# angeladai/sgnn

Measured on AMD Instinct MI355X. Metric: TSDF blocks/sec fwd+bwd (64^3@5% occ, bs32), higher is better.
Workload: dtype f32

## Files before the change

### include/sgnn_hip.h

```cpp
#ifndef SGNN_HIP_H
#define SGNN_HIP_H

#include <stdint.h>

#ifdef __cplusplus
extern "C" {
#endif

#define SGNN_OK 0
#define SGNN_EINVAL (-1)
#define SGNN_EHIP (-2)
#define SGNN_EOVERFLOW (-3)
#define SGNN_ENOWS (-4)

#define SGNN_STATUS_COORD_RANGE 1
#define SGNN_STATUS_DUPLICATE 2
#define SGNN_STATUS_OVERFLOW 4

typedef void *sgnn_stream_t;

const char *sgnn_last_error(void);
int sgnn_version(void);
const char *sgnn_arch(void);

// ... 40 lines not shown

#define SGNN_RULEBOOK_MULTI_MAX 4
int sgnn_rulebook_subm3_multi(int count, const uint64_t *const *keys, const int32_t *const *vals, const int64_t *caps,
                              const int32_t *const *coords, const int64_t *ns, int32_t *const *nbrs, const int64_t *lds,
                              const int64_t *const *n_devs, sgnn_stream_t stream);

int sgnn_rulebook_subm3_dense(const uint64_t *keys, const int32_t *vals, int64_t cap, const int32_t *coords, int64_t n,
                              int dim_z, int dim_y, int dim_x, int32_t *volume, int64_t volume_entries, int32_t *nbr,
                              int64_t ld, const int64_t *n_dev, sgnn_stream_t stream);
int sgnn_rulebook_subm3_volume(const int32_t *coords, int64_t n, int dim_z, int dim_y, int dim_x, int32_t *volume,
                               int64_t volume_entries, int32_t *nbr, int64_t ld, const int64_t *n_dev, int32_t *status,
                               sgnn_stream_t stream);

int64_t sgnn_down2_ws_bytes(int64_t nf);
int sgnn_rulebook_down2(const int32_t *fine_coords, int64_t nf, uint64_t *ckeys, int32_t *cvals,
                        int64_t ccap, int32_t *parent, int32_t *coarse_coords, int64_t *n_coarse,
                        void *ws, int64_t ws_bytes, sgnn_stream_t stream);
int sgnn_down2_tables(const int32_t *fine_coords, const int32_t *parent, int64_t nf,
                      int32_t *children, int64_t ldc, int64_t nc, int32_t *ptable, int64_t ldf,
                      const int64_t *nf_dev, const int64_t *nc_dev, sgnn_stream_t stream);

int64_t sgnn_down2_chain_ws_bytes(int64_t cap);
int sgnn_down2_chain(const int32_t *fine_coords, int64_t n0, const int64_t *n0_dev, int64_t cap, int depth,
                     void *const *ckeys, void *const *cvals, int64_t ccap, void *const *parent,
                     void *const *coarse_coords, int64_t *counts_dev, const int64_t *level_caps, int32_t *status,
                     void *ws, int64_t ws_bytes, sgnn_stream_t stream);

int64_t sgnn_down2_chain_tables_ws_bytes(int64_t cap, int depth);
int sgnn_down2_chain_tables(const int32_t *fine_coords, const int64_t *n0_dev, int64_t cap, int depth,
                            void *const *ckeys, void *const *cvals, int64_t ccap, void *const *parent,
                            void *const *coarse_coords, int64_t *counts_dev, const int64_t *level_caps,
                            void *const *children, void *const *ptable, int32_t *status, void *ws, int64_t ws_bytes,
                            sgnn_stream_t stream);

#define SGNN_CONV_TRANSPOSE_W 1
#define SGNN_CONV_FLIP_K 2
int sgnn_conv_fwd(const float *x, int64_t n_in, int cin, const float *w, int K, const int32_t *table,
                  int64_t ld, int64_t n_out, int cout, float *y, int flags, int in_shift,
                  sgnn_stream_t stream);

int sgnn_conv_fwd_ex(const float *x, int64_t n_in, int cin, const float *w, int K, const int32_t *table,
                     int64_t ld, int64_t n_out, int cout, float *y, int flags, int in_shift,
                     const int32_t *kmap, const int32_t *kadd, int in_mul, int groups, int table_rows,
                     sgnn_stream_t stream);
int sgnn_conv_bwd_weight_ex(const float *x, int64_t n_in, int cin, const float *dy, int cout,
                            const int32_t *table, int64_t ld, int K, int64_t n_out, float *dw, int in_shift,
                            const int32_t *kmap, const int32_t *kadd, int in_mul, int groups, int table_rows,
                            void *ws, int64_t ws_bytes, sgnn_stream_t stream);

int64_t sgnn_conv_stats_blocks(int64_t n_out);
int sgnn_conv_fwd_epi(const float *x, int64_t n_in, int cin, int64_t ldx, const float *w, int K,
                      const int32_t *table, int64_t ld, int64_t n_out, int cout, float *y, int64_t ldy, int flags,
                      const float *addend, int64_t ld_add, int stats, double *partial, const float *bn_x,
                      int64_t ld_bnx, const float *mean, const float *invstd, const float *gamma, const float *beta,
                      float leak, sgnn_stream_t stream);

int64_t sgnn_conv_bwd_weight_ws_bytes(int64_t n_out, int K, int cin, int cout);
int sgnn_conv_bwd_weight(const float *x, int64_t n_in, int cin, const float *dy, int cout,
                         const int32_t *table, int64_t ld, int K, int64_t n_out, float *dw, int in_shift, void *ws,
                         int64_t ws_bytes, sgnn_stream_t stream);

int sgnn_expand_weights(const float *w, int cin, int cout, float *wc, sgnn_stream_t stream);
int sgnn_expand_weights_bwd(const float *dwc, int cin, int cout, float *dw, sgnn_stream_t stream);

int64_t sgnn_bn_ws_bytes(int64_t n, int c);
int sgnn_bn_fwd(const float *x, int64_t n, int c, const float *gamma, const float *beta,
// ... 334 lines not shown
```

### sgnn_amd/_lib.py

```python
import ctypes
import os

import torch

_HERE = os.path.dirname(os.path.abspath(__file__))
LIB_PATH = os.environ.get('SGNN_LIB') or os.path.join(_HERE, 'lib', 'libsgnn_hip.so')

c_i32, c_i64, c_f32, c_vp, c_cp = ctypes.c_int, ctypes.c_int64, ctypes.c_float, ctypes.c_void_p, ctypes.c_char_p

PROTOTYPES = {
    'sgnn_last_error': (c_cp, []),
    'sgnn_version': (c_i32, []),
    'sgnn_arch': (c_cp, []),
    'sgnn_tune_set': (c_i64, [c_cp, c_i64]),
    'sgnn_tune_get': (c_i64, [c_cp]),
    'sgnn_tune_names': (c_cp, []),
    'sgnn_tune_current': (c_vp, []),
    'sgnn_hash_capacity': (c_i64, [c_i64]),
    'sgnn_coords_from_i64': (c_i32, [c_vp, c_i64, c_vp, c_vp, c_vp, c_vp]),
    'sgnn_coords_to_i64': (c_i32, [c_vp, c_i64, c_vp, c_vp, c_vp]),
    'sgnn_hash_build': (c_i32, [c_vp, c_i64, c_vp, c_vp, c_i64, c_vp, c_vp, c_vp]),
    'sgnn_hash_lookup': (c_i32, [c_vp, c_vp, c_i64, c_vp, c_i64, c_vp, c_vp, c_vp]),
    'sgnn_rulebook_subm3': (c_i32, [c_vp, c_vp, c_i64, c_vp, c_i64, c_vp, c_i64, c_vp, c_vp]),
    'sgnn_rulebook_subm3_multi': (c_i32, [c_i32, c_vp, c_vp, c_vp, c_vp, c_vp, c_vp, c_vp, c_vp, c_vp]),
    'sgnn_rulebook_subm3_dense': (c_i32, [c_vp, c_vp, c_i64, c_vp, c_i64, c_i32, c_i32, c_i32, c_vp, c_i64, c_vp, c_i64, c_vp, c_vp]),
    'sgnn_rulebook_subm3_volume': (c_i32, [c_vp, c_i64, c_i32, c_i32, c_i32, c_vp, c_i64, c_vp, c_i64, c_vp, c_vp, c_vp]),
    'sgnn_down2_ws_bytes': (c_i64, [c_i64]),
    'sgnn_rulebook_down2': (c_i32, [c_vp, c_i64, c_vp, c_vp, c_i64, c_vp, c_vp, c_vp, c_vp, c_i64, c_vp]),
    'sgnn_down2_chain_ws_bytes': (c_i64, [c_i64]),
    'sgnn_down2_chain': (c_i32, [c_vp, c_i64, c_vp, c_i64, c_i32, c_vp, c_vp, c_i64, c_vp, c_vp, c_vp, c_vp, c_vp, c_vp, c_i64, c_vp]),
    'sgnn_down2_chain_tables_ws_bytes': (c_i64, [c_i64, c_i32]),
    'sgnn_down2_chain_tables': (c_i32, [c_vp, c_vp, c_i64, c_i32, c_vp, c_vp, c_i64, c_vp, c_vp, c_vp, c_vp, c_vp, c_vp, c_vp, c_vp,
                                        c_i64, c_vp]),
    'sgnn_down2_tables': (c_i32, [c_vp, c_vp, c_i64, c_vp, c_i64, c_i64, c_vp, c_i64, c_vp, c_vp, c_vp]),
    'sgnn_conv_fwd': (c_i32, [c_vp, c_i64, c_i32, c_vp, c_i32, c_vp, c_i64, c_i64, c_i32, c_vp, c_i32, c_i32, c_vp]),
    'sgnn_conv_fwd_ex': (c_i32, [c_vp, c_i64, c_i32, c_vp, c_i32, c_vp, c_i64, c_i64, c_i32, c_vp, c_i32, c_i32, c_vp, c_vp, c_i32, c_i32, c_i32, c_vp]),
    'sgnn_conv_bwd_weight_ex': (c_i32, [c_vp, c_i64, c_i32, c_vp, c_i32, c_vp, c_i64, c_i32, c_i64, c_vp, c_i32, c_vp, c_vp, c_i32, c_i32, c_i32, c_vp, c_i64, c_vp]),
    'sgnn_conv_stats_blocks': (c_i64, [c_i64]),
    'sgnn_conv_fwd_epi': (c_i32, [c_vp, c_i64, c_i32, c_i64, c_vp, c_i32, c_vp, c_i64, c_i64, c_i32, c_vp, c_i64, c_i32, c_vp, c_i64, c_i32, c_vp, c_vp, c_i64, c_vp, c_vp, c_vp, c_vp, c_f32, c_vp]),
    'sgnn_conv_bwd_weight_ws_bytes': (c_i64, [c_i64, c_i32, c_i32, c_i32]),
    'sgnn_conv_bwd_weight': (c_i32, [c_vp, c_i64, c_i32, c_vp, c_i32, c_vp, c_i64, c_i32, c_i64, c_vp, c_i32, c_vp, c_i64, c_vp]),
    'sgnn_bn_ws_bytes': (c_i64, [c_i64, c_i32]),
    'sgnn_bn_fwd': (c_i32, [c_vp, c_i64, c_i32, c_vp, c_vp, c_vp, c_vp, c_f32, c_f32, c_i32, c_f32, c_vp, c_vp, c_vp, c_vp, c_i64, c_vp]),
    'sgnn_bn_bwd': (c_i32, [c_vp, c_vp, c_i64, c_i32, c_vp, c_vp, c_vp, c_vp, c_i32, c_f32, c_vp, c_vp, c_vp, c_vp, c_i64, c_vp]),
    'sgnn_bn_bwd_add': (c_i32, [c_vp, c_vp, c_i64, c_i32, c_vp, c_vp, c_vp, c_vp, c_i32, c_f32, c_vp, c_vp, c_vp, c_vp, c_vp, c_i64, c_vp]),
    'sgnn_bn_fwd_ex': (c_i32, [c_vp, c_i64, c_i64, c_i32, c_vp, c_vp, c_vp, c_vp, c_f32, c_f32, c_i32, c_f32, c_vp, c_vp, c_vp, c_i64, c_vp, c_i64, c_vp, c_i64, c_vp]),
    'sgnn_bn_bwd_ex': (c_i32, [c_vp, c_i64, c_vp, c_i64, c_i64, c_i32, c_vp, c_vp, c_vp, c_vp, c_i32, c_f32, c_vp, c_i64, c_vp, c_i64, c_vp, c_vp, c_vp, c_i64, c_vp, c_i64, c_vp]),
    'sgnn_copy_multi': (c_i32, [c_vp, c_vp, c_vp, c_i32, c_vp]),
    'sgnn_gather_rows': (c_i32, [c_vp, c_i32, c_vp, c_i64, c_vp, c_vp]),
    'sgnn_gather_rows_dn': (c_i32, [c_vp, c_i32, c_vp, c_vp, c_i64, c_vp, c_vp]),
    'sgnn_scatter_rows': (c_i32, [c_vp, c_i32, c_vp, c_i64, c_vp, c_i64, c_vp, c_vp]),
    'sgnn_gather_sum': (c_i32, [c_vp, c_i32, c_vp, c_i64, c_i32, c_i64, c_vp, c_vp]),
    'sgnn_repeat_rows': (c_i32, [c_vp, c_i32, c_i64, c_i32, c_vp, c_vp]),
    'sgnn_sum_groups': (c_i32, [c_vp, c_i32, c_i64, c_i32, c_vp, c_vp]),
    'sgnn_concat_rows': (c_i32, [c_vp, c_i32, c_vp, c_vp, c_i32, c_vp, c_i64, c_vp, c_vp]),
    'sgnn_concat_rows_bwd': (c_i32, [c_vp, c_i32, c_vp, c_i32, c_vp, c_i64, c_vp, c_i64, c_vp, c_i64, c_vp]),
    'sgnn_add': (c_i32, [c_vp, c_vp, c_i64, c_vp, c_vp]),
    'sgnn_expand8_coords': (c_i32, [c_vp, c_i64, c_vp, c_vp, c_vp]),
    'sgnn_expand8_coords_i64': (c_i32, [c_vp, c_i64, c_vp, c_vp, c_vp, c_vp]),
    'sgnn_dense_coords': (c_i32, [c_i32, c_i32, c_i32, c_i32, c_vp, c_vp]),
    'sgnn_compact_ws_bytes': (c_i64, [c_i64]),
    'sgnn_compact_sigmoid': (c_i32, [c_vp, c_i64, c_i64, c_vp, c_vp, c_vp, c_i64, c_vp]),
    'sgnn_compact_dense': (c_i32, [c_vp, c_i64, c_vp, c_i32, c_i32, c_i32, c_i32, c_vp, c_vp, c_vp, c_i64, c_vp]),
    'sgnn_compact_mask': (c_i32, [c_vp, c_i64, c_vp, c_vp, c_vp, c_i64, c_vp]),
    'sgnn_compact_sigmoid_cap': (c_i32, [c_vp, c_i64, c_i64, c_vp, c_vp, c_vp, c_i64, c_vp, c_vp, c_i64, c_vp]),
    'sgnn_compact_dense_cap': (c_i32, [c_vp, c_i64, c_vp, c_vp, c_i32, c_i32, c_i32, c_i32, c_vp, c_vp, c_i64, c_vp, c_vp, c_i64, c_vp]),
# ... 226 lines not shown
```

### sgnn_amd/csrc/grid_rules.hip

```cpp
#include <stdarg.h>
#include "common.h"

static thread_local char g_err[512] = "";

void sgnn_set_error(const char *fmt, ...) {
  va_list ap;
  va_start(ap, fmt);
  vsnprintf(g_err, sizeof(g_err), fmt, ap);
  va_end(ap);
}

SGNN_EXPORT const char *sgnn_last_error(void) { return g_err; }
SGNN_EXPORT int sgnn_version(void) { return 100; }
SGNN_EXPORT const char *sgnn_arch(void) { return "gfx950"; }

SGNN_EXPORT int64_t sgnn_hash_capacity(int64_t n) {
  const int64_t want = 4 * n < 262144 ? 4 * n : (2 * n > 262144 ? 2 * n : 262144);
  int64_t cap = 1024;
  while (cap < want) cap <<= 1;
  return cap;
}

__global__ __launch_bounds__(256) void k_coords_from_i64(const int64_t *__restrict__ locs, int64_t n,
                                                        int4 *__restrict__ coords, int32_t *status,
// ... 690 lines not shown
}

#define CHAIN_MAX_DEPTH 8

struct ChainScratch {
  int32_t *slot_of, *rank_at, *owner;
};

static int64_t chain_ws_bytes(int64_t cap, int64_t ccap, int slices) {
  const int64_t nblk = (cap + SCAN_BLOCK - 1) / SCAN_BLOCK;
  return (slices * (2 * cap + ccap) + nblk + 1) * (int64_t)sizeof(int32_t) + 256;
}

static int32_t *chain_ws_carve(void *ws, int64_t cap, int64_t ccap, int slices, ChainScratch *w) {
  int32_t *p = (int32_t *)ws;
  for (int l = 0; l < slices; ++l, p += 2 * cap + ccap) w[l] = ChainScratch{p, p + cap, p + 2 * cap};
  return p;
}

struct ChainInit {
  unsigned long long *ckeys[CHAIN_MAX_DEPTH];
  int32_t *owner[CHAIN_MAX_DEPTH];
  int32_t *rank_at[CHAIN_MAX_DEPTH];
  int64_t ccap, cap;
};

__device__ __forceinline__ void chain_init_rows(unsigned long long *__restrict__ ckeys, int32_t *__restrict__ owner,
                                                int64_t ccap, int32_t *__restrict__ rank_at, int64_t cap) {
  const int64_t stride = (int64_t)gridDim.x * 256;
  const int64_t top = ccap > cap ? ccap : cap;
  for (int64_t i = (int64_t)blockIdx.x * 256 + threadIdx.x; i < top; i += stride) {
    if (i < ccap) {
      ckeys[i] = ~0ull;
      owner[i] = 0x7FFFFFFF;
    }
    if (i < cap) rank_at[i] = -1;
  }
}

__global__ __launch_bounds__(256) void k_chain_init(unsigned long long *__restrict__ ckeys, int32_t *__restrict__ owner,
                                                   int64_t ccap, int32_t *__restrict__ rank_at, int64_t cap) {
  chain_init_rows(ckeys, owner, ccap, rank_at, cap);
}

__global__ __launch_bounds__(256) void k_chain_init_all(ChainInit a) {
  chain_init_rows(a.ckeys[blockIdx.y], a.owner[blockIdx.y], a.ccap, a.rank_at[blockIdx.y], a.cap);
}

__device__ __forceinline__ void chain_insert_rows(const int4 *__restrict__ fine, const int64_t *n_dev, int64_t n_host,
                                                  unsigned long long *__restrict__ ckeys,
                                                  int32_t *__restrict__ owner, uint64_t mask,
                                                  int32_t *__restrict__ slot_of) {
  const int64_t nf = sgnn_dyn_n(n_host, n_dev);
  int64_t i = (int64_t)blockIdx.x * 256 + threadIdx.x;
  const int64_t stride = (int64_t)gridDim.x * 256;
  for (; i < nf; i += stride) {
    const int4 c = fine[i];
    const uint64_t key = sgnn_pack_key(c.x >> 1, c.y >> 1, c.z >> 1, c.w);
    uint64_t slot = sgnn_hash64(key) & mask;
    while (true) {
      const unsigned long long prev = atomicCAS(&ckeys[slot], SGNN_EMPTY_KEY, (unsigned long long)key);
      if (prev == SGNN_EMPTY_KEY || prev == key) break;
      slot = (slot + 1) & mask;
    }
    atomicMin(&owner[slot], (int32_t)i);
    slot_of[i] = (int32_t)slot;
  }
}

// ... 124 lines not shown
  for (; i < iend; i += stride) {
    if (Tables && i >= nf) {
      down2_table_row<false>(i, true, fine, -1, nc, nullptr, children, ldc, ptable, ldf);
      continue;
    }
    const int32_t sl = slot_of[i];
    const int32_t p = rank_at[owner[sl]];
    if (rank_at[i] >= 0) cvals[sl] = p;
    if (Tables) down2_table_row<true>(i, false, fine, p, nc, parent, children, ldc, ptable, ldf);
    else parent[i] = p;
  }
}

__global__ __launch_bounds__(256) void k_chain_parent(const int64_t *n_dev, int64_t n_host,
                                                     const int32_t *__restrict__ owner,
                                                     const int32_t *__restrict__ rank_at,
                                                     const int32_t *__restrict__ slot_of,
                                                     int32_t *__restrict__ parent, int32_t *__restrict__ cvals) {
  chain_parent_rows<false>(nullptr, n_dev, n_host, owner, rank_at, slot_of, parent, cvals, nullptr, 0, nullptr, 0, nullptr, 0);
}

__global__ __launch_bounds__(256) void k_chain_parent_tables(ChainTables t) {
  chain_parent_rows<true>(t.fine, t.n_dev, t.n_host, t.owner, t.rank_at, t.slot_of, t.parent, t.cvals, t.nc_dev, t.nc_cap,
                          t.children, t.ldc, t.ptable, t.ldf);
}

__global__ __launch_bounds__(256) void k_chain_tables_insert(ChainTables t, unsigned long long *__restrict__ ckeys_next,
                                                            int32_t *__restrict__ owner_next, uint64_t mask,
                                                            int32_t *__restrict__ slot_of_next, const int4 *coarse,
                                                            int64_t n_host_next) {
  chain_parent_rows<true>(t.fine, t.n_dev, t.n_host, t.owner, t.rank_at, t.slot_of, t.parent, t.cvals, t.nc_dev, t.nc_cap,
                          t.children, t.ldc, t.ptable, t.ldf);
  chain_insert_rows(coarse, t.nc_dev, n_host_next, ckeys_next, owner_next, mask, slot_of_next);
}

static void chain_launch_init(const ChainInit &ini, int levels, hipStream_t s) {
  SGNN_LAUNCH(k_chain_init_all, dim3(sgnn_grid_for(ini.ccap, 256, 4096), levels), dim3(256), 0, s, ini);
}

static void chain_launch_insert(const int4 *fine, const int64_t *n_dev, int64_t n_host, int64_t cap, void *ckeys,
                                const ChainScratch &w, int64_t ccap, hipStream_t s) {
  SGNN_LAUNCH(k_chain_insert, dim3(sgnn_grid_for(cap, 256, 8192)), dim3(256), 0, s, fine, n_dev, n_host,
              (unsigned long long *)ckeys, w.owner, (uint64_t)(ccap - 1), w.slot_of);
}

static ScanInline chain_launch_count(const ChainScratch &w, const int64_t *n_dev, int64_t n_host, int64_t cap,
                                     int32_t *block_sums, int64_t *count, const ScanLimit &lim, hipStream_t s) {
  const int64_t nblk = (cap + SCAN_BLOCK - 1) / SCAN_BLOCK;
  SGNN_LAUNCH((k_scan_count<FlagOwner>), dim3((unsigned)nblk), dim3(256), 0, s, FlagOwner{w.slot_of, w.owner}, n_host,
              block_sums, n_dev);
  if (scan_inline_ok(nblk)) return ScanInline{nblk, count, lim};
  SGNN_LAUNCH(k_scan_block_sums, dim3(1), dim3(1024), 0, s, block_sums, nblk, count, lim);
  return kNoInline;
}

SGNN_EXPORT int64_t sgnn_down2_ws_bytes(int64_t nf) { return chain_ws_bytes(nf, sgnn_hash_capacity(nf), 1); }
SGNN_EXPORT int64_t sgnn_down2_chain_ws_bytes(int64_t cap) { return chain_ws_bytes(cap, sgnn_hash_capacity(cap), 1); }
SGNN_EXPORT int64_t sgnn_down2_chain_tables_ws_bytes(int64_t cap, int depth) {
  return chain_ws_bytes(cap, sgnn_hash_capacity(cap), depth);
}

static int chain_hip_result(const char *who, hipError_t e) {
  if (e == hipSuccess) return SGNN_OK;
  sgnn_set_error("%s: HIP error: %s", who, hipGetErrorString(e));
  return SGNN_EHIP;
}
// ... 34 lines not shown
                (const int32_t *)w.rank_at, (const int32_t *)w.slot_of, (int32_t *)parent[l], (int32_t *)cvals[l]);
    fine = (const int4 *)coarse_coords[l];
    n_dev = counts_dev + l;
    n_host = cap;
  }
  return chain_hip_result(who, hipGetLastError());
}

SGNN_EXPORT int sgnn_rulebook_down2(const int32_t *fine_coords, int64_t nf, uint64_t *ckeys, int32_t *cvals,
                                    int64_t ccap, int32_t *parent, int32_t *coarse_coords,
                                    int64_t *n_coarse, void *ws, int64_t ws_bytes, sgnn_stream_t stream) {
  SGNN_CHECK_ARG(nf >= 0 && n_coarse && ckeys && cvals);
  SGNN_CHECK_ARG(ccap >= 2 * nf && ccap >= 2 && (ccap & (ccap - 1)) == 0 && ccap < (1ll << 31));
  SGNN_CHECK_ARG(nf == 0 || (fine_coords && parent && coarse_coords));
  void *const k = ckeys, *const v = cvals, *const p = parent, *const c = coarse_coords;
  return down2_chain("sgnn_rulebook_down2", fine_coords, nf, nullptr, nf, 1, &k, &v, ccap, &p, &c, n_coarse, nullptr,
                     nullptr, ws, ws_bytes, (hipStream_t)stream);
}

SGNN_EXPORT int sgnn_down2_chain(const int32_t *fine_coords, int64_t n0, const int64_t *n0_dev, int64_t cap, int depth,
                                 void *const *ckeys, void *const *cvals, int64_t ccap, void *const *parent,
                                 void *const *coarse_coords, int64_t *counts_dev, const int64_t *level_caps,
                                 int32_t *status, void *ws, int64_t ws_bytes, sgnn_stream_t stream) {
  SGNN_CHECK_ARG(!level_caps || status);
  SGNN_CHECK_ARG(depth >= 1 && depth <= CHAIN_MAX_DEPTH && cap >= 0 && n0 >= 0 && n0 <= cap && counts_dev && ckeys &&
                 cvals && parent && coarse_coords);
  SGNN_CHECK_ARG(ccap >= 2 * cap && ccap >= 2 && (ccap & (ccap - 1)) == 0 && ccap < (1ll << 31));
  for (int l = 0; l < depth; ++l) SGNN_CHECK_ARG(ckeys[l] && (cap == 0 || (cvals[l] && parent[l] && coarse_coords[l])));
  SGNN_CHECK_ARG(cap == 0 || fine_coords);
  return down2_chain("sgnn_down2_chain", fine_coords, n0, n0_dev, cap, depth, ckeys, cvals, ccap, parent, coarse_coords,
                     counts_dev, level_caps, status, ws, ws_bytes, (hipStream_t)stream);
}

SGNN_EXPORT int sgnn_down2_chain_tables(const int32_t *fine_coords, const int64_t *n0_dev, int64_t cap, int depth,
                                        void *const *ckeys, void *const *cvals, int64_t ccap, void *const *parent,
                                        void *const *coarse_coords, int64_t *counts_dev, const int64_t *level_caps,
                                        void *const *children, void *const *ptable, int32_t *status, void *ws,
                                        int64_t ws_bytes, sgnn_stream_t stream) {
  hipStream_t s = (hipStream_t)stream;
  SGNN_CHECK_ARG(depth >= 1 && depth <= CHAIN_MAX_DEPTH && cap >= 1 && n0_dev && counts_dev && level_caps && status &&
                 ckeys && cvals && parent && coarse_coords && children && ptable && fine_coords);
  SGNN_CHECK_ARG(ccap >= 2 * cap && ccap >= 2 && (ccap & (ccap - 1)) == 0 && ccap < (1ll << 31));
  if (!ws || ws_bytes < chain_ws_bytes(cap, ccap, depth)) {
    sgnn_set_error("sgnn_down2_chain_tables: workspace too small");
    return SGNN_ENOWS;
  }
  ChainScratch w[CHAIN_MAX_DEPTH];
  int32_t *block_sums = chain_ws_carve(ws, cap, ccap, depth, w);
  ChainInit ini{};
  for (int l = 0; l < depth; ++l) {
    SGNN_CHECK_ARG(ckeys[l] && cvals[l] && parent[l] && coarse_coords[l] && children[l] && ptable[l] && level_caps[l] >= 1);
    ini.ckeys[l] = (unsigned long long *)ckeys[l];
    ini.owner[l] = w[l].owner;
    ini.rank_at[l] = w[l].rank_at;
  }
  ini.ccap = ccap;
  ini.cap = cap;
  chain_launch_init(ini, depth, s);
  const int4 *fine = (const int4 *)fine_coords;
  const int64_t *n_dev = n0_dev;
  int64_t fine_cap = cap;
  const int g = sgnn_grid_for(cap, 256, 8192);
  const bool merged = g_tune.chain_merged != 0;
  for (int l = 0; l < depth; ++l) {
    const int64_t ccap_l = level_caps[l] < cap ? level_caps[l] : cap;
    const int64_t ldc = ((ccap_l + 255) / 256) * 256, ldf = ((fine_cap + 255) / 256) * 256;
    if (l == 0 || !merged)
      chain_launch_insert(fine, n_dev, cap, cap, ckeys[l], w[l], ccap, s);
    const ScanInline si = chain_launch_count(w[l], n_dev, cap, cap, block_sums, counts_dev + l,
                                             ScanLimit{ccap_l, nullptr, 0, status}, s);
    SGNN_LAUNCH(k_chain_emit2, dim3((unsigned)((cap + SCAN_BLOCK - 1) / SCAN_BLOCK)), dim3(256), 0, s, fine,
                (const int32_t *)w[l].slot_of, (const int32_t *)w[l].owner, n_dev, cap, (const int32_t *)block_sums,
                (int4 *)coarse_coords[l], w[l].rank_at, (const int64_t *)(counts_dev + l), (int32_t *)children[l], ldc, si);
    const ChainTables t{fine, n_dev, cap, w[l].owner, w[l].rank_at, w[l].slot_of, (int32_t *)parent[l], (int32_t *)cvals[l],
                        counts_dev + l, ccap_l, (int32_t *)children[l], ldc, (int32_t *)ptable[l], ldf};
    if (merged && l + 1 < depth)
      SGNN_LAUNCH(k_chain_tables_insert, dim3(g), dim3(256), 0, s, t, (unsigned long long *)ckeys[l + 1], w[l + 1].owner,
                  (uint64_t)(ccap - 1), w[l + 1].slot_of, (const int4 *)coarse_coords[l], cap);
    else
      SGNN_LAUNCH(k_chain_parent_tables, dim3(g), dim3(256), 0, s, t);
    fine = (const int4 *)coarse_coords[l];
    n_dev = counts_dev + l;
    fine_cap = ccap_l;
  }
  SGNN_CHECK_LAUNCH();
  return SGNN_OK;
}

__global__ __launch_bounds__(256) void k_down2_tables(const int4 *__restrict__ fine,
                                                     const int32_t *__restrict__ parent, int64_t nf,
                                                     int32_t *__restrict__ children, int64_t ldc,
                                                     int32_t *__restrict__ ptable, int64_t ldf, int64_t nc,
                                                     const int64_t *nf_dev, const int64_t *nc_dev) {
  nf = sgnn_dyn_n(nf, nf_dev);
  nc = sgnn_dyn_n(nc, nc_dev);
  int64_t i = (int64_t)blockIdx.x * 256 + threadIdx.x;
  const int64_t stride = (int64_t)gridDim.x * 256;
  const int64_t iend = pad_end(nf, ldf);
  for (; i < iend; i += stride) {
    if (i >= nf)
      down2_table_row<false>(i, true, fine, -1, nc, nullptr, children, ldc, ptable, ldf);
    else
      down2_table_row<false>(i, false, fine, parent[i], nc, nullptr, children, ldc, ptable, ldf);
  }
}

SGNN_EXPORT int sgnn_down2_tables(const int32_t *fine_coords, const int32_t *parent, int64_t nf,
                                  int32_t *children, int64_t ldc, int64_t nc, int32_t *ptable, int64_t ldf,
                                  const int64_t *nf_dev, const int64_t *nc_dev, sgnn_stream_t stream) {
  hipStream_t s = (hipStream_t)stream;
  SGNN_CHECK_ARG(nf >= 0 && nc >= 0 && ldc >= nc && ldf >= nf);
  if (nc > 0) {
    SGNN_CHECK_ARG(children);
    if (nc_dev)
      SGNN_LAUNCH(k_fill_rows_dyn, dim3(sgnn_grid_for(8 * nc, 256, 4096)), dim3(256), 0, s, children, 8, ldc, nc, nc_dev);
    else
      if (sgnn_fill32(children, 0xFFFFFFFFu, 8 * ldc, s) != SGNN_OK) return SGNN_EHIP;
  }
  if (nf == 0) return SGNN_OK;
// ... 83 lines not shown
```

### sgnn_amd/model.py

```python
import os

import numpy as np
import torch
import torch.nn as nn
import torch.nn.functional as F

from . import scn
from .scn import functions as F_
from .scn import program as P_
from .scn.metadata import coords_from_locs
from .scn.sites import info, attach


STAGES = True
TEACHER_GEOMETRY_FIRST = os.environ.get('SGNN_TEACHER_GEOMETRY_FIRST', '1') != '0'


def _k4s2_maps():
    P, S = [], []
    for g in range(8):
        j = (g >> 2, (g >> 1) & 1, g & 1)
        for i_ in range(8):
            i = (i_ >> 2, (i_ >> 1) & 1, i_ & 1)
            k = [3 - 2 * i[a] - j[a] for a in range(3)]
# ... 587 lines not shown
        R = len(self.refinement)
        plan = F_.compact_sigmoid_plan(geo.coords, 2, int(geo.coords.shape[0]), geo.coords, 2 if runs[0] else 0, teacher[0])
        plans = [plan]
        for h in range(R):
            if not runs[h] or plan[1] == 0:
                plans.append(None)
                continue
            locs = plan[2]
            children = F_.expand8_coords(locs)
            attach(locs, children=children)
            plan = F_.compact_sigmoid_plan(children, 2, 8 * plan[1], children,
                                           self.refinement[h].plan_depth, teacher[h + 1])
            plans.append(plan)
        return plans

    def _forward_stages(self, feat_rows, occ_rows, skips, geo, loss_weights, runs, teacher=None, plans=None,
                        capacity=None):
        if not (self.pass_occ or self.pass_feats):
            return None
        R = len(self.refinement)
        if getattr(geo, 'coords_i64', None) is None:
            geo.coords_i64 = F_.coords_to_i64(geo.coords)
        outputs = [[geo.coords_i64, occ_rows]]
        n_all = occ_rows.shape[0]
        tv = (lambda h: None) if teacher is None else (lambda h: teacher[h])
        if plans is not None:
            sel, cnt, locs = plans[0]
        elif capacity is not None:
            sel, cnt, locs = F_.compact_capped(occ_rows.detach(), 2, n_all, geo.coords, 2 if runs[0] else 0, capacity, 0,
                                               tv(0))
        else:
            sel, cnt, locs = F_.compact_sigmoid_plan(occ_rows.detach(), 2, n_all, geo.coords, 2 if runs[0] else 0, tv(0))
        prev = (occ_rows if self.pass_occ else None, feat_rows if self.pass_feats else None, sel, locs, cnt)
        for h in range(R):
            if not runs[h]:
                outputs.append([[], []])
                continue
            if cnt == 0:
                outputs.append([[], []])
                continue
            ref = self.refinement[h]
            got = ref.stage(prev, skips[R - h] if self.use_skip_sparse else None)
            if got is None:
                return None if h == 0 else self._stage_fallback()
            y, out, coords_next = got
            outputs.append([F_.coords_to_i64(coords_next), out])
            if plans is not None:
                sel, cnt, locs = plans[h + 1]
            elif capacity is not None:
                sel, cnt, locs = F_.compact_capped(out.detach(), 2, out.shape[0], coords_next, ref.plan_depth, capacity,
                                                   h + 1, tv(h + 1))
            else:
                sel, cnt, locs = F_.compact_sigmoid_plan(out.detach(), 2, out.shape[0], coords_next, ref.plan_depth, tv(h + 1))
            prev = (y if ref.pass_feats else None, out if ref.pass_occ else None, sel, locs, cnt)
        if not runs[R]:
            return [[], []], outputs
        if cnt == 0:
            return [[], []], outputs
        sdf = self.surfacepred.stage(prev, skips[0] if self.use_skip_sparse else None)
        if sdf is None:
            return self._stage_fallback()
        return [F_.coords_to_i64(prev[3]), sdf], outputs

    @staticmethod
    def _stage_fallback():
        raise RuntimeError('sgnn_amd: a generative stage could not be compiled into a native program after an earlier '
                           'one was; set sgnn_amd.model.STAGES = False to run the per-module path')
```

### sgnn_amd/scn/functions.py

```python
import torch
from torch.autograd import Function

from .. import _lib
from .._lib import ptr
from .metadata import runtime
from .sites import info, attach

import os

CONV_TRANSPOSE_W = 1
CONV_FLIP_K = 2
FUSED_GLUE = os.environ.get('SGNN_FUSED_GLUE', '1') != '0'


_ws_cache = {}


def _ws_bytes(name, *args):
    k = (name,) + args
    v = _ws_cache.get(k)
    if v is None:
        if len(_ws_cache) > 4096:
            _ws_cache.clear()
        v = _ws_cache[k] = _lib.query(name, *args)
# ... 483 lines not shown
def compact_sigmoid_plan(logits, stride, n, coords_all, depth, teacher=None):
    from . import metadata as MD
    rt = runtime(logits.device)
    if not MD.CHAIN or depth < 1 or n == 0:
        if teacher is None:
            sel, cnt = compact_sigmoid(logits, stride, n)
        else:
            sel = torch.empty(max(n, 1), dtype=torch.int32, device=logits.device)
            wsb = _lib.query('sgnn_compact_ws_bytes', n)
            _compact_call(logits, stride, n, coords_all, sel, rt, rt.workspace(wsb), wsb, teacher)
            cnt = rt.read_count()
            sel = sel[:cnt]
        if MD.COUNT_LOG is not None:
            MD.COUNT_LOG.append(('gen', int(cnt), []))
        return sel, cnt, gather_coords(coords_all, sel, cnt)
    sel = torch.empty(n, dtype=torch.int32, device=logits.device)
    wsb = _lib.query('sgnn_compact_ws_bytes', n)
    ws = rt.workspace(wsb)
    _compact_call(logits, stride, n, coords_all, sel, rt, ws, wsb, teacher)
    locs_cap = torch.empty(n, 4, dtype=torch.int32, device=logits.device)
    _lib.call('sgnn_gather_rows_dn', ptr(coords_all), 4, ptr(sel), ptr(rt.state), n, ptr(locs_cap))
    _inherit_bounds(locs_cap, coords_all)
    chain = MD.PendingChain(locs_cap, 0, True, depth)
    host = rt.read_counts()
    count = int(host[0])
    locs = _inherit_bounds(locs_cap[:count], coords_all)
    if MD.COUNT_LOG is not None:
        MD.COUNT_LOG.append(('gen', count, [int(v) for v in host[2:2 + chain.depth]]))
    if count:
        attach(locs, plan=chain.finalize(count, host))
    return sel[:count], count, locs


def compact_capped(logits, stride, n_all, coords_all, depth, capacity, g, teacher=None):
    from . import metadata as MD
    dev = coords_all.device
    rt = runtime(dev)
    K, pyr_caps = capacity.gen[g]
    cnt2 = capacity.kept2(g)
    n_cnt = info(coords_all).cnt
    sel = torch.empty(max(n_all, 1), dtype=torch.int32, device=dev)
    wsb = _lib.query('sgnn_compact_ws_bytes', n_all)
    ws = rt.workspace(wsb)
    kept, kept8 = cnt2[0:1], cnt2[1:2]
    locs = _inherit_bounds(torch.empty(K, 4, dtype=torch.int32, device=dev), coords_all)
    if FUSED_GLUE:
        if teacher is None:
            _lib.call('sgnn_compact_sigmoid_cap_locs', ptr(logits), stride, n_all, ptr(n_cnt), ptr(coords_all), ptr(sel),
                      ptr(locs), ptr(cnt2), K, ptr(rt.status32), ptr(ws), wsb)
        else:
            B, _, d0, d1, d2 = (int(v) for v in teacher.shape)
            _lib.call('sgnn_compact_dense_cap_locs', ptr(coords_all), n_all, ptr(n_cnt), ptr(teacher), B, d0, d1, d2,
                      ptr(sel), ptr(locs), ptr(cnt2), K, ptr(rt.status32), ptr(ws), wsb)
    else:
        if teacher is None:
            _lib.call('sgnn_compact_sigmoid_cap', ptr(logits), stride, n_all, ptr(n_cnt), ptr(sel), ptr(cnt2), K,
                      ptr(rt.status32), ptr(ws), wsb)
        else:
            B, _, d0, d1, d2 = (int(v) for v in teacher.shape)
            _lib.call('sgnn_compact_dense_cap', ptr(coords_all), n_all, ptr(n_cnt), ptr(teacher), B, d0, d1, d2, ptr(sel),
                      ptr(cnt2), K, ptr(rt.status32), ptr(ws), wsb)
        _lib.call('sgnn_gather_rows_dn', ptr(coords_all), 4, ptr(sel), ptr(kept), K, ptr(locs))
    attach(locs, cnt=kept, cnt8=kept8)
    if depth >= 1:
        depth = min(depth, len(pyr_caps))
        chain = MD.PendingChain(locs, K, True, depth, n0_cnt=kept, counts=capacity.pyr_counts(g, depth),
                                level_caps=pyr_caps)
        attach(locs, plan=chain.finalize_capped())
    return sel, K, locs


def compact_mask(mask_u8, n):
    rt = runtime(mask_u8.device)
    sel = torch.empty(max(n, 1), dtype=torch.int32, device=mask_u8.device)
    wsb = _lib.query('sgnn_compact_ws_bytes', n)
    ws = rt.workspace(wsb)
    _lib.call('sgnn_compact_mask', ptr(mask_u8), n, ptr(sel), ptr(rt.state), ptr(ws), wsb)
    count = rt.read_count()
    return sel[:count], count


def _inherit_bounds(coords, parent, scale=1):
    b = info(parent).bounds
    if b is not None:
        attach(coords, bounds=(int(b[0]), int(b[1]) * scale, int(b[2]) * scale, int(b[3]) * scale))
    return coords


def gather_coords(coords32, sel, m):
    out = torch.empty(m, 4, dtype=torch.int32, device=coords32.device)
    _lib.call('sgnn_gather_rows', ptr(coords32), 4, ptr(sel), m, ptr(out))
    return _inherit_bounds(out, coords32)


def expand8_coords(coords32, with_i64=False):
    n = coords32.shape[0]
    out = torch.empty(8 * n, 4, dtype=torch.int32, device=coords32.device)
    parent = info(coords32)
    cnt, o64 = parent.cnt, None
    if with_i64 and FUSED_GLUE:
# ... 27 lines not shown
```

### sgnn_amd/scn/metadata.py

```python
import numpy as np
import os
import threading
from contextlib import nullcontext as _nullcontext

import torch

from .. import _lib
from .._lib import ptr
from .sites import info, attach, carry


SIDE_LANE = os.environ.get('SGNN_SIDE_LANE', '1') != '0'
SIDE_PRIORITY = int(os.environ.get('SGNN_SIDE_PRIORITY', '0'))
SIDE_PYRAMID = os.environ.get('SGNN_SIDE_PYRAMID', '1') != '0'
PYRAMID_LANE = 2


class _Runtime(object):

    def __init__(self, device):
        self.device = device
        self.ws = torch.empty(1 << 20, dtype=torch.uint8, device=device)
        self.state = torch.zeros(8, dtype=torch.int64, device=device)
        self.status32 = self.state[1:2].view(torch.int32)
        self.syncs = 0

    def index_volume(self):
        if getattr(self, '_volume', None) is None:
            self._volume = torch.full((INDEX_VOLUME_ENTRIES,), -1, dtype=torch.int32, device=self.device)
        return self._volume

    def workspace(self, nbytes):
        if self.ws.numel() < nbytes:
            self.ws = torch.empty(int(nbytes * 1.5) + 256, dtype=torch.uint8, device=self.device)
        return self.ws

    def pyramid_stream(self):
        if getattr(self, '_side_stream', None) is None:
            self._side_stream = torch.cuda.Stream(device=self.device, priority=SIDE_PRIORITY)
            self._side_ws = None
        self._pyr_stream = self._side_stream
        return self._pyr_stream

    def side_lane(self, nbytes):
        if not SIDE_LANE:
            if getattr(self, '_side_on', False):
                _lib.query('sgnn_prog_set_side_stream', None, None, 0)
                self._side_on = False
# ... 154 lines not shown
        return out if self.cnt is None else attach(out, cnt=self.cnt)


class Down2(object):
    ready = None

    def __init__(self, fine, coarse, parent, children, ldc, ptable, ldf):
        self.fine, self.coarse = fine, coarse
        self.parent, self.children, self.ldc, self.ptable, self.ldf = parent, children, ldc, ptable, ldf


def build_down2(fine):
    rt = runtime(fine.device)
    nf, dev = fine.n, fine.device
    ccap = _lib.query('sgnn_hash_capacity', nf)
    ckeys = torch.empty(ccap, dtype=torch.int64, device=dev)
    cvals = torch.empty(ccap, dtype=torch.int32, device=dev)
    parent = torch.empty(max(nf, 1), dtype=torch.int32, device=dev)
    ccoords = torch.empty(max(nf, 1), 4, dtype=torch.int32, device=dev)
    wsb = _lib.query('sgnn_down2_ws_bytes', nf)
    ws = rt.workspace(wsb)
    _lib.call('sgnn_rulebook_down2', ptr(fine.coords), nf, ptr(ckeys), ptr(cvals), ccap, ptr(parent), ptr(ccoords),
              ptr(rt.state), ptr(ws), wsb)
    nc = rt.read_count()
    return _down2_tables(fine, Grid(ccoords[:nc], ckeys, cvals, ccap), parent)


CHAIN = True
MAX_CHAIN = 6


class PendingChain(object):

    def __init__(self, coords_cap, n0, n0_on_device, depth, n0_cnt=None, counts=None, level_caps=None):
        dev = coords_cap.device
        rt = runtime(dev)
        cap = int(coords_cap.shape[0])
        depth = min(depth, MAX_CHAIN)
        self.n0_cnt, self.counts, self.level_caps = n0_cnt, counts, level_caps
        self.coords_cap, self.cap, self.depth = coords_cap, cap, depth
        self.ccap = _lib.query('sgnn_hash_capacity', cap)
        mk = lambda shape, dt: torch.empty(shape, dtype=dt, device=dev)
        self.ckeys = [mk(self.ccap, torch.int64) for _ in range(depth)]
        self.cvals = [mk(self.ccap, torch.int32) for _ in range(depth)]
        self.parent = [mk(max(cap, 1), torch.int32) for _ in range(depth)]
        self.ccoords = [mk((max(cap, 1), 4), torch.int32) for _ in range(depth)]
        wsb = _lib.query('sgnn_down2_chain_ws_bytes', cap)
        ws = rt.workspace(wsb)
        arr = lambda ts: np.ascontiguousarray(np.array([t.data_ptr() for t in ts], dtype=np.uint64))
        self._keep = [arr(self.ckeys), arr(self.cvals), arr(self.parent), arr(self.ccoords)]
        if counts is not None:
            assert n0_cnt is not None and level_caps is not None and len(level_caps) >= depth and counts.numel() >= depth
            caps = [min(int(c), cap) for c in level_caps[:depth]]
            caps_np = np.ascontiguousarray(np.array(caps, dtype=np.int64))
            ld = [_round_up(max(cap, 1), 256)] + [_round_up(max(c, 1), 256) for c in caps]
            self.children = [mk(8 * ld[l + 1], torch.int32) for l in range(depth)]
            self.ptable = [mk(8 * ld[l], torch.int32) for l in range(depth)]
            self._keep += [arr(self.children), arr(self.ptable)]
            wsb = _lib.query('sgnn_down2_chain_tables_ws_bytes', cap, depth)
            self.side = None
            if SIDE_PYRAMID:
                self.side = rt.pyramid_stream()
                with lane(PYRAMID_LANE):
                    rt2 = runtime(dev)
                    if rt2.ws.numel() < wsb:
                        self.side.synchronize()
                    ws = rt2.workspace(wsb)
                _lib.stamp('fork')
                self.side.wait_stream(torch.cuda.current_stream(dev))
            else:
                ws = rt.workspace(wsb)
            with (torch.cuda.stream(self.side) if self.side is not None else _nullcontext()):
                _lib.stamp('lane<')
                _lib.call('sgnn_down2_chain_tables', ptr(coords_cap), ptr(n0_cnt), cap, depth,
                          self._keep[0].ctypes.data, self._keep[1].ctypes.data, self.ccap, self._keep[2].ctypes.data,
                          self._keep[3].ctypes.data, ptr(counts), caps_np.ctypes.data, self._keep[4].ctypes.data,
                          self._keep[5].ctypes.data, ptr(rt.status32), ptr(ws), wsb)
            return
        _lib.call('sgnn_down2_chain', ptr(coords_cap), 0 if n0_on_device else int(n0),
                  rt.state.data_ptr() if n0_on_device else None, cap, depth, self._keep[0].ctypes.data,
                  self._keep[1].ctypes.data, self.ccap, self._keep[2].ctypes.data, self._keep[3].ctypes.data,
                  rt.state.data_ptr() + 16, None, None, ptr(ws), wsb)

    def finalize(self, n0, host_state):
        counts = [int(v) for v in host_state[2:2 + self.depth]]
        fine = Grid(self.coords_cap[:n0])
        fine.bounds = info(self.coords_cap).bounds
        grid0, downs = fine, []
        for l in range(self.depth):
            nc = counts[l]
            coarse = Grid(self.ccoords[l][:nc], self.ckeys[l], self.cvals[l], self.ccap)
            downs.append(_down2_tables(fine, coarse, self.parent[l]))
            fine = coarse
        return grid0, downs

    def finalize_capped(self, grid0=None):
        fine = grid0 if grid0 is not None else Grid(self.coords_cap, cnt=self.n0_cnt)
        grid0, downs = fine, []
        for l in range(self.depth):
            cap_l = min(int(self.level_caps[l]), self.cap)
            coarse = Grid(self.ccoords[l][:cap_l], self.ckeys[l], self.cvals[l], self.ccap, cnt=self.counts[l:l + 1])
            assert coarse.ld * 8 == self.children[l].numel() and fine.ld * 8 == self.ptable[l].numel()
            downs.append(Down2(fine, coarse, self.parent[l][:fine.n], self.children[l], coarse.ld, self.ptable[l], fine.ld))
            fine = coarse
        if getattr(self, 'side', None) is not None:
            for d in downs:
                g = d.coarse
                g._nbr = torch.empty(27 * g.ld, dtype=torch.int32, device=g.device)
            with torch.cuda.stream(self.side):
                for i in range(0, len(downs), _lib.RULEBOOK_MULTI_MAX):
# ... 125 lines not shown
```

Before: 5803.

## Build coarse pyramid levels from sorted coords via sibling-flag scan instead of hashing

Adds a sorted path for the down2 chain-table builder. When fine coordinates are known to be sorted so that siblings are contiguous, parents are found with a neighbour-compare flag, a block scan and a compacting emit, instead of a hash insert, owner election and rank scatter. The hash table is still filled per level for later lookups, but without contention. The path is enabled by default for capped compaction generations and relies on the generation count to assume sortedness, so it gives wrong results if that ordering assumption ever fails.

```diff
diff --git a/include/sgnn_hip.h b/include/sgnn_hip.h
--- a/include/sgnn_hip.h
+++ b/include/sgnn_hip.h
@@ -96,6 +96,12 @@
                             void *const *coarse_coords, int64_t *counts_dev, const int64_t *level_caps,
                             void *const *children, void *const *ptable, int32_t *status, void *ws, int64_t ws_bytes,
                             sgnn_stream_t stream);
+
+int sgnn_down2_chain_tables_sorted(const int32_t *fine_coords, const int64_t *n0_dev, int64_t cap, int depth,
+                                   void *const *ckeys, void *const *cvals, int64_t ccap, void *const *parent,
+                                   void *const *coarse_coords, int64_t *counts_dev, const int64_t *level_caps,
+                                   void *const *children, void *const *ptable, int32_t *status, void *ws, int64_t ws_bytes,
+                                   int sorted_levels, sgnn_stream_t stream);
 
 #define SGNN_CONV_TRANSPOSE_W 1
 #define SGNN_CONV_FLIP_K 2
diff --git a/sgnn_amd/_lib.py b/sgnn_amd/_lib.py
--- a/sgnn_amd/_lib.py
+++ b/sgnn_amd/_lib.py
@@ -32,6 +32,8 @@
     'sgnn_down2_chain_tables_ws_bytes': (c_i64, [c_i64, c_i32]),
     'sgnn_down2_chain_tables': (c_i32, [c_vp, c_vp, c_i64, c_i32, c_vp, c_vp, c_i64, c_vp, c_vp, c_vp, c_vp, c_vp, c_vp, c_vp, c_vp,
                                         c_i64, c_vp]),
+    'sgnn_down2_chain_tables_sorted': (c_i32, [c_vp, c_vp, c_i64, c_i32, c_vp, c_vp, c_i64, c_vp, c_vp, c_vp, c_vp, c_vp, c_vp, c_vp,
+                                               c_vp, c_i64, c_i32, c_vp]),
     'sgnn_down2_tables': (c_i32, [c_vp, c_vp, c_i64, c_vp, c_i64, c_i64, c_vp, c_i64, c_vp, c_vp, c_vp]),
     'sgnn_conv_fwd': (c_i32, [c_vp, c_i64, c_i32, c_vp, c_i32, c_vp, c_i64, c_i64, c_i32, c_vp, c_i32, c_i32, c_vp]),
     'sgnn_conv_fwd_ex': (c_i32, [c_vp, c_i64, c_i32, c_vp, c_i32, c_vp, c_i64, c_i64, c_i32, c_vp, c_i32, c_i32, c_vp, c_vp, c_i32, c_i32, c_i32, c_vp]),
diff --git a/sgnn_amd/csrc/grid_rules.hip b/sgnn_amd/csrc/grid_rules.hip
--- a/sgnn_amd/csrc/grid_rules.hip
+++ b/sgnn_amd/csrc/grid_rules.hip
@@ -746,9 +746,9 @@
   for (int64_t i = (int64_t)blockIdx.x * 256 + threadIdx.x; i < top; i += stride) {
     if (i < ccap) {
       ckeys[i] = ~0ull;
-      owner[i] = 0x7FFFFFFF;
-    }
-    if (i < cap) rank_at[i] = -1;
+      if (owner) owner[i] = 0x7FFFFFFF;
+    }
+    if (rank_at && i < cap) rank_at[i] = -1;
   }
 }
 
@@ -939,6 +939,93 @@
   chain_parent_rows<true>(t.fine, t.n_dev, t.n_host, t.owner, t.rank_at, t.slot_of, t.parent, t.cvals, t.nc_dev, t.nc_cap,
                           t.children, t.ldc, t.ptable, t.ldf);
   chain_insert_rows(coarse, t.nc_dev, n_host_next, ckeys_next, owner_next, mask, slot_of_next);
+}
+
+struct FlagSibling {
+  const int4 *fine;
+  static __device__ __forceinline__ uint64_t parent_key(const int4 c) {
+    return sgnn_pack_key(c.x >> 1, c.y >> 1, c.z >> 1, c.w);
+  }
+  __device__ __forceinline__ bool operator()(int64_t i) const {
+    return i == 0 || parent_key(fine[i]) != parent_key(fine[i - 1]);
+  }
+};
+
+__global__ __launch_bounds__(256) void k_chain_emit_sorted(const int4 *__restrict__ fine, const int64_t *n_dev,
+                                                          int64_t n_host, const int32_t *block_offsets,
+                                                          int4 *__restrict__ coarse, int32_t *__restrict__ parent,
+                                                          const int64_t *nc_dev, int32_t *__restrict__ children,
+                                                          int64_t ldc, ScanInline si) {
+  __shared__ int lds[8];
+  const int64_t n = sgnn_dyn_n(n_host, n_dev);
+  int running = 0;
+  int64_t nc_live;
+  if (si.nblk > 0) {
+    int64_t total;
+    scan_offsets_inline(block_offsets, si.nblk, blockIdx.x, lds, running, total);
+    nc_live = scan_publish(total, si.count, si.lim, blockIdx.x == 0 && threadIdx.x == 0);
+  } else {
+    nc_live = sgnn_dyn_n(ldc, nc_dev);
+  }
+  {
+    const int64_t end = pad_end(nc_live, ldc);
+    const int64_t total = end * 8, stride = (int64_t)gridDim.x * 256;
+    for (int64_t g = (int64_t)blockIdx.x * 256 + threadIdx.x; g < total; g += stride) children[(g / end) * ldc + (g % end)] = -1;
+  }
+  const int64_t base = (int64_t)blockIdx.x * SCAN_BLOCK;
+  if (base >= n) return;
+  if (si.nblk <= 0) running = block_offsets[blockIdx.x];
+#pragma unroll 1
+  for (int it = 0; it < SCAN_ITEMS; ++it) {
+    const int64_t i = base + it * 256 + threadIdx.x;
+    const bool live = i < n;
+    int4 c = make_int4(0, 0, 0, 0);
+    uint64_t key = 0;
+    bool f = false;
+    if (live) {
+      c = fine[i];
+      key = FlagSibling::parent_key(c);
+      f = i == 0 || key != FlagSibling::parent_key(fine[i - 1]);
+    }
+    int total;
+    const int r = sgnn_block_rank256(f, lds, total);
+    if (live) {
+      const int32_t rank = running + r - (f ? 0 : 1);
+      parent[i] = rank;
+      if (f) coarse[rank] = make_int4(c.x >> 1, c.y >> 1, c.z >> 1, c.w);
+    }
+    running += total;
+  }
+}
+
+__global__ __launch_bounds__(256) void k_chain_tables_sorted(ChainTables t, unsigned long long *__restrict__ ckeys,
+                                                            unsigned long long *__restrict__ ckeys_next,
+                                                            int32_t *__restrict__ owner_next, uint64_t mask,
+                                                            int32_t *__restrict__ slot_of_next, const int4 *coarse,
+                                                            int64_t n_host_next) {
+  const int64_t nf = sgnn_dyn_n(t.n_host, t.n_dev);
+  const int64_t nc = sgnn_dyn_n(t.nc_cap, t.nc_dev);
+  const int64_t iend = pad_end(nf, t.ldf);
+  const int64_t stride = (int64_t)gridDim.x * 256;
+  for (int64_t i = (int64_t)blockIdx.x * 256 + threadIdx.x; i < iend; i += stride) {
+    if (i >= nf)
+      down2_table_row<false>(i, true, t.fine, -1, nc, nullptr, t.children, t.ldc, t.ptable, t.ldf);
+    else {
+      const int32_t p = t.parent[i];
+      const uint64_t key = FlagSibling::parent_key(t.fine[i]);
+      if (i == 0 || key != FlagSibling::parent_key(t.fine[i - 1])) {
+        uint64_t slot = sgnn_hash64(key) & mask;
+        while (true) {
+          const unsigned long long prev = atomicCAS(&ckeys[slot], SGNN_EMPTY_KEY, (unsigned long long)key);
+          if (prev == SGNN_EMPTY_KEY || prev == key) break;
+          slot = (slot + 1) & mask;
+        }
+        t.cvals[slot] = p;
+      }
+      down2_table_row<true>(i, false, t.fine, p, nc, t.parent, t.children, t.ldc, t.ptable, t.ldf);
+    }
+  }
+  if (ckeys_next) chain_insert_rows(coarse, t.nc_dev, n_host_next, ckeys_next, owner_next, mask, slot_of_next);
 }
 
 static void chain_launch_init(const ChainInit &ini, int levels, hipStream_t s) {
@@ -1039,27 +1126,35 @@
                      counts_dev, level_caps, status, ws, ws_bytes, (hipStream_t)stream);
 }
 
-SGNN_EXPORT int sgnn_down2_chain_tables(const int32_t *fine_coords, const int64_t *n0_dev, int64_t cap, int depth,
-                                        void *const *ckeys, void *const *cvals, int64_t ccap, void *const *parent,
-                                        void *const *coarse_coords, int64_t *counts_dev, const int64_t *level_caps,
-                                        void *const *children, void *const *ptable, int32_t *status, void *ws,
-                                        int64_t ws_bytes, sgnn_stream_t stream) {
-  hipStream_t s = (hipStream_t)stream;
-  SGNN_CHECK_ARG(depth >= 1 && depth <= CHAIN_MAX_DEPTH && cap >= 1 && n0_dev && counts_dev && level_caps && status &&
-                 ckeys && cvals && parent && coarse_coords && children && ptable && fine_coords);
-  SGNN_CHECK_ARG(ccap >= 2 * cap && ccap >= 2 && (ccap & (ccap - 1)) == 0 && ccap < (1ll << 31));
+#define CHAIN_CHECK_ARG(cond)                                        \
+  do {                                                               \
+    if (!(cond)) {                                                   \
+      sgnn_set_error("%s: invalid argument: %s", who, #cond);        \
+      return SGNN_EINVAL;                                            \
+    }                                                                \
+  } while (0)
+
+static int down2_chain_tables(const char *who, const int32_t *fine_coords, const int64_t *n0_dev, int64_t cap, int depth,
+                              void *const *ckeys, void *const *cvals, int64_t ccap, void *const *parent,
+                              void *const *coarse_coords, int64_t *counts_dev, const int64_t *level_caps,
+                              void *const *children, void *const *ptable, int32_t *status, void *ws, int64_t ws_bytes,
+                              hipStream_t s, int sorted_levels) {
+  CHAIN_CHECK_ARG(depth >= 1 && depth <= CHAIN_MAX_DEPTH && cap >= 1 && n0_dev && counts_dev && level_caps && status &&
+                  ckeys && cvals && parent && coarse_coords && children && ptable && fine_coords);
+  CHAIN_CHECK_ARG(ccap >= 2 * cap && ccap >= 2 && (ccap & (ccap - 1)) == 0 && ccap < (1ll << 31));
+  CHAIN_CHECK_ARG(sorted_levels >= 0 && sorted_levels <= depth);
   if (!ws || ws_bytes < chain_ws_bytes(cap, ccap, depth)) {
-    sgnn_set_error("sgnn_down2_chain_tables: workspace too small");
+    sgnn_set_error("%s: workspace too small", who);
     return SGNN_ENOWS;
   }
   ChainScratch w[CHAIN_MAX_DEPTH];
   int32_t *block_sums = chain_ws_carve(ws, cap, ccap, depth, w);
   ChainInit ini{};
   for (int l = 0; l < depth; ++l) {
-    SGNN_CHECK_ARG(ckeys[l] && cvals[l] && parent[l] && coarse_coords[l] && children[l] && ptable[l] && level_caps[l] >= 1);
+    CHAIN_CHECK_ARG(ckeys[l] && cvals[l] && parent[l] && coarse_coords[l] && children[l] && ptable[l] && level_caps[l] >= 1);
     ini.ckeys[l] = (unsigned long long *)ckeys[l];
-    ini.owner[l] = w[l].owner;
-    ini.rank_at[l] = w[l].rank_at;
+    ini.owner[l] = l < sorted_levels ? nullptr : w[l].owner;
+    ini.rank_at[l] = l < sorted_levels ? nullptr : w[l].rank_at;
   }
   ini.ccap = ccap;
   ini.cap = cap;
@@ -1072,26 +1167,64 @@
   for (int l = 0; l < depth; ++l) {
     const int64_t ccap_l = level_caps[l] < cap ? level_caps[l] : cap;
     const int64_t ldc = ((ccap_l + 255) / 256) * 256, ldf = ((fine_cap + 255) / 256) * 256;
-    if (l == 0 || !merged)
-      chain_launch_insert(fine, n_dev, cap, cap, ckeys[l], w[l], ccap, s);
-    const ScanInline si = chain_launch_count(w[l], n_dev, cap, cap, block_sums, counts_dev + l,
-                                             ScanLimit{ccap_l, nullptr, 0, status}, s);
-    SGNN_LAUNCH(k_chain_emit2, dim3((unsigned)((cap + SCAN_BLOCK - 1) / SCAN_BLOCK)), dim3(256), 0, s, fine,
-                (const int32_t *)w[l].slot_of, (const int32_t *)w[l].owner, n_dev, cap, (const int32_t *)block_sums,
-                (int4 *)coarse_coords[l], w[l].rank_at, (const int64_t *)(counts_dev + l), (int32_t *)children[l], ldc, si);
-    const ChainTables t{fine, n_dev, cap, w[l].owner, w[l].rank_at, w[l].slot_of, (int32_t *)parent[l], (int32_t *)cvals[l],
-                        counts_dev + l, ccap_l, (int32_t *)children[l], ldc, (int32_t *)ptable[l], ldf};
-    if (merged && l + 1 < depth)
-      SGNN_LAUNCH(k_chain_tables_insert, dim3(g), dim3(256), 0, s, t, (unsigned long long *)ckeys[l + 1], w[l + 1].owner,
-                  (uint64_t)(ccap - 1), w[l + 1].slot_of, (const int4 *)coarse_coords[l], cap);
-    else
-      SGNN_LAUNCH(k_chain_parent_tables, dim3(g), dim3(256), 0, s, t);
+    const ScanLimit lim{ccap_l, nullptr, 0, status};
+    const bool ride = merged && l + 1 < depth;
+    if (l < sorted_levels) {
+      const int64_t nblk = (cap + SCAN_BLOCK - 1) / SCAN_BLOCK;
+      SGNN_LAUNCH((k_scan_count<FlagSibling>), dim3((unsigned)nblk), dim3(256), 0, s, FlagSibling{fine}, cap, block_sums, n_dev);
+      ScanInline si = kNoInline;
+      if (scan_inline_ok(nblk)) si = ScanInline{nblk, counts_dev + l, lim};
+      else SGNN_LAUNCH(k_scan_block_sums, dim3(1), dim3(1024), 0, s, block_sums, nblk, counts_dev + l, lim);
+      SGNN_LAUNCH(k_chain_emit_sorted, dim3((unsigned)nblk), dim3(256), 0, s, fine, n_dev, cap, (const int32_t *)block_sums,
+                  (int4 *)coarse_coords[l], (int32_t *)parent[l], (const int64_t *)(counts_dev + l), (int32_t *)children[l],
+                  ldc, si);
+      const ChainTables t{fine, n_dev, cap, nullptr, nullptr, nullptr, (int32_t *)parent[l], (int32_t *)cvals[l],
+                          counts_dev + l, ccap_l, (int32_t *)children[l], ldc, (int32_t *)ptable[l], ldf};
+      const bool hash_next = ride && l + 1 >= sorted_levels;
+      SGNN_LAUNCH(k_chain_tables_sorted, dim3(g), dim3(256), 0, s, t, (unsigned long long *)ckeys[l], hash_next ? (unsigned long long *)ckeys[l + 1] : nullptr,
+                  w[l + 1 < depth ? l + 1 : l].owner, (uint64_t)(ccap - 1), w[l + 1 < depth ? l + 1 : l].slot_of,
+                  (const int4 *)coarse_coords[l], cap);
+    } else {
+      if (l == 0 || !merged)
+        chain_launch_insert(fine, n_dev, cap, cap, ckeys[l], w[l], ccap, s);
+      const ScanInline si = chain_launch_count(w[l], n_dev, cap, cap, block_sums, counts_dev + l, lim, s);
+      SGNN_LAUNCH(k_chain_emit2, dim3((unsigned)((cap + SCAN_BLOCK - 1) / SCAN_BLOCK)), dim3(256), 0, s, fine,
+                  (const int32_t *)w[l].slot_of, (const int32_t *)w[l].owner, n_dev, cap, (const int32_t *)block_sums,
+                  (int4 *)coarse_coords[l], w[l].rank_at, (const int64_t *)(counts_dev + l), (int32_t *)children[l], ldc, si);
+      const ChainTables t{fine, n_dev, cap, w[l].owner, w[l].rank_at, w[l].slot_of, (int32_t *)parent[l], (int32_t *)cvals[l],
+                          counts_dev + l, ccap_l, (int32_t *)children[l], ldc, (int32_t *)ptable[l], ldf};
+      if (ride)
+        SGNN_LAUNCH(k_chain_tables_insert, dim3(g), dim3(256), 0, s, t, (unsigned long long *)ckeys[l + 1], w[l + 1].owner,
+                    (uint64_t)(ccap - 1), w[l + 1].slot_of, (const int4 *)coarse_coords[l], cap);
+      else
+        SGNN_LAUNCH(k_chain_parent_tables, dim3(g), dim3(256), 0, s, t);
+    }
     fine = (const int4 *)coarse_coords[l];
     n_dev = counts_dev + l;
     fine_cap = ccap_l;
   }
-  SGNN_CHECK_LAUNCH();
-  return SGNN_OK;
+  return chain_hip_result(who, hipGetLastError());
+}
+#undef CHAIN_CHECK_ARG
+
+SGNN_EXPORT int sgnn_down2_chain_tables(const int32_t *fine_coords, const int64_t *n0_dev, int64_t cap, int depth,
+                                        void *const *ckeys, void *const *cvals, int64_t ccap, void *const *parent,
+                                        void *const *coarse_coords, int64_t *counts_dev, const int64_t *level_caps,
+                                        void *const *children, void *const *ptable, int32_t *status, void *ws,
+                                        int64_t ws_bytes, sgnn_stream_t stream) {
+  return down2_chain_tables("sgnn_down2_chain_tables", fine_coords, n0_dev, cap, depth, ckeys, cvals, ccap, parent,
+                            coarse_coords, counts_dev, level_caps, children, ptable, status, ws, ws_bytes,
+                            (hipStream_t)stream, 0);
+}
+
+SGNN_EXPORT int sgnn_down2_chain_tables_sorted(const int32_t *fine_coords, const int64_t *n0_dev, int64_t cap, int depth,
+                                               void *const *ckeys, void *const *cvals, int64_t ccap, void *const *parent,
+                                               void *const *coarse_coords, int64_t *counts_dev, const int64_t *level_caps,
+                                               void *const *children, void *const *ptable, int32_t *status, void *ws,
+                                               int64_t ws_bytes, int sorted_levels, sgnn_stream_t stream) {
+  return down2_chain_tables("sgnn_down2_chain_tables_sorted", fine_coords, n0_dev, cap, depth, ckeys, cvals, ccap, parent,
+                            coarse_coords, counts_dev, level_caps, children, ptable, status, ws, ws_bytes,
+                            (hipStream_t)stream, sorted_levels);
 }
 
 __global__ __launch_bounds__(256) void k_down2_tables(const int4 *__restrict__ fine,
diff --git a/sgnn_amd/model.py b/sgnn_amd/model.py
--- a/sgnn_amd/model.py
+++ b/sgnn_amd/model.py
@@ -643,6 +643,7 @@
         else:
             sel, cnt, locs = F_.compact_sigmoid_plan(occ_rows.detach(), 2, n_all, geo.coords, 2 if runs[0] else 0, tv(0))
         prev = (occ_rows if self.pass_occ else None, feat_rows if self.pass_feats else None, sel, locs, cnt)
+        gens = 0
         for h in range(R):
             if not runs[h]:
                 outputs.append([[], []])
@@ -659,8 +660,9 @@
             if plans is not None:
                 sel, cnt, locs = plans[h + 1]
             elif capacity is not None:
+                gens += 1
                 sel, cnt, locs = F_.compact_capped(out.detach(), 2, out.shape[0], coords_next, ref.plan_depth, capacity,
-                                                   h + 1, tv(h + 1))
+                                                   h + 1, tv(h + 1), generations=gens)
             else:
                 sel, cnt, locs = F_.compact_sigmoid_plan(out.detach(), 2, out.shape[0], coords_next, ref.plan_depth, tv(h + 1))
             prev = (y if ref.pass_feats else None, out if ref.pass_occ else None, sel, locs, cnt)
diff --git a/sgnn_amd/scn/functions.py b/sgnn_amd/scn/functions.py
--- a/sgnn_amd/scn/functions.py
+++ b/sgnn_amd/scn/functions.py
@@ -539,7 +539,7 @@
     return sel[:count], count, locs
 
 
-def compact_capped(logits, stride, n_all, coords_all, depth, capacity, g, teacher=None):
+def compact_capped(logits, stride, n_all, coords_all, depth, capacity, g, teacher=None, generations=0):
     from . import metadata as MD
     dev = coords_all.device
     rt = runtime(dev)
@@ -572,7 +572,7 @@
     if depth >= 1:
         depth = min(depth, len(pyr_caps))
         chain = MD.PendingChain(locs, K, True, depth, n0_cnt=kept, counts=capacity.pyr_counts(g, depth),
-                                level_caps=pyr_caps)
+                                level_caps=pyr_caps, generations=generations)
         attach(locs, plan=chain.finalize_capped())
     return sel, K, locs
 
diff --git a/sgnn_amd/scn/metadata.py b/sgnn_amd/scn/metadata.py
--- a/sgnn_amd/scn/metadata.py
+++ b/sgnn_amd/scn/metadata.py
@@ -14,6 +14,7 @@
 SIDE_PRIORITY = int(os.environ.get('SGNN_SIDE_PRIORITY', '0'))
 SIDE_PYRAMID = os.environ.get('SGNN_SIDE_PYRAMID', '1') != '0'
 PYRAMID_LANE = 2
+CHAIN_SORTED = os.environ.get('SGNN_CHAIN_SORTED', '1') != '0'
 
 
 class _Runtime(object):
@@ -234,13 +235,14 @@
 
 class PendingChain(object):
 
-    def __init__(self, coords_cap, n0, n0_on_device, depth, n0_cnt=None, counts=None, level_caps=None):
+    def __init__(self, coords_cap, n0, n0_on_device, depth, n0_cnt=None, counts=None, level_caps=None, generations=0):
         dev = coords_cap.device
         rt = runtime(dev)
         cap = int(coords_cap.shape[0])
         depth = min(depth, MAX_CHAIN)
         self.n0_cnt, self.counts, self.level_caps = n0_cnt, counts, level_caps
         self.coords_cap, self.cap, self.depth = coords_cap, cap, depth
+        self.sorted_levels = min(int(generations), depth) if (CHAIN_SORTED and counts is not None) else 0
         self.ccap = _lib.query('sgnn_hash_capacity', cap)
         mk = lambda shape, dt: torch.empty(shape, dtype=dt, device=dev)
         self.ckeys = [mk(self.ccap, torch.int64) for _ in range(depth)]
@@ -274,10 +276,10 @@
                 ws = rt.workspace(wsb)
             with (torch.cuda.stream(self.side) if self.side is not None else _nullcontext()):
                 _lib.stamp('lane<')
-                _lib.call('sgnn_down2_chain_tables', ptr(coords_cap), ptr(n0_cnt), cap, depth,
+                _lib.call('sgnn_down2_chain_tables_sorted', ptr(coords_cap), ptr(n0_cnt), cap, depth,
                           self._keep[0].ctypes.data, self._keep[1].ctypes.data, self.ccap, self._keep[2].ctypes.data,
                           self._keep[3].ctypes.data, ptr(counts), caps_np.ctypes.data, self._keep[4].ctypes.data,
-                          self._keep[5].ctypes.data, ptr(rt.status32), ptr(ws), wsb)
+                          self._keep[5].ctypes.data, ptr(rt.status32), ptr(ws), wsb, self.sorted_levels)
             return
         _lib.call('sgnn_down2_chain', ptr(coords_cap), 0 if n0_on_device else int(n0),
                   rt.state.data_ptr() if n0_on_device else None, cap, depth, self._keep[0].ctypes.data,
```

Result: no change. 5839, median of 6 (+0.6%).
